# FueledByRedBull/audio-forge

Hardware: AMD Instinct MI355X
Metric: 48 kHz mono frames/s (real-time-factor x streams), voice chain (higher is better)
Workload: dtype f64

## Files before the change

audio-forge_amd/csrc/af_api.cpp:

```cpp
#include <hip/hip_runtime.h>

#include <algorithm>
#include <cmath>
#include <cstdio>
#include <cstdlib>
#include <cstring>
#include <limits>
#include <memory>
#include <string>
#include <utility>
#include <vector>

#include "af_api_internal.hpp"
#include "af_device.h"
#include "af_host.hpp"
#include "af_mixdown_host.hpp"
#include "af_output_writer_host.hpp"
#include "af_resampler_host.hpp"
#include "af_retune.h"
#include "af_stages.h"
#include "af_suppressor_host.hpp"
#include "af_switches.hpp"

namespace af {
// ... 327 lines not shown
    export_params(e);
    if (e->proto.limiter_enabled &&
        af::quad_kernel_dynamic_lds(e->host_params.n_eq_sections, e->proto.limiter.lookahead_samples, true) > af::kMaxLdsBytes)
      return fail(AF_ERR_UNSUPPORTED, "limiter lookahead of %d samples exceeds what the LDS-resident ring holds",
                  e->proto.limiter.lookahead_samples);
    if (e->proto.compressor_enabled && e->proto.compressor.auto_makeup_enabled) {
      if (e->host_params.comp.meter_slots <= 0)
        return fail(AF_ERR_UNSUPPORTED, "auto-makeup needs a control block that divides the 400 ms loudness window "
                                        "(e.g. 480 or 960 samples at 48 kHz) and a sample rate the meter supports");
      if (e->host_params.control_block < 64)
        return fail(AF_ERR_UNSUPPORTED, "auto-makeup needs control blocks of at least 64 samples");
    }
    if (!e->extra_presets.empty()) {
      for (const af_preset &ps : e->extra_presets) {
        if (ps.host_params.control_block != e->host_params.control_block)
          return fail(AF_ERR_INVALID_ARGUMENT, "every preset of an engine must use the same control block");
        if (ps.proto.sample_rate != e->proto.sample_rate) return fail(AF_ERR_INVALID_ARGUMENT, "presets must share the sample rate");
      }
      if (e->kernel != AF_KERNEL_AUTO && e->kernel != AF_KERNEL_PHASED && e->kernel != AF_KERNEL_STAGED)
        return fail(AF_ERR_UNSUPPORTED, "multi-preset engines run the token-ring kernel or the stage pipeline");
      const size_t n_groups = (size_t)(e->n_streams + 63) / 64;
      if (e->group_preset.size() != n_groups) e->group_preset.assign(n_groups, 0);
      e->d_group_preset.release();
      e->d_params_multi.release();
      AF_HIP(e->d_group_preset.reserve_exact(sizeof(int32_t) * n_groups));
      AF_HIP(hipMemcpy(e->d_group_preset, e->group_preset.data(), sizeof(int32_t) * n_groups, hipMemcpyHostToDevice));
      AF_HIP(e->d_params_multi.reserve_exact(sizeof(af::ChainParams) * (1 + e->extra_presets.size())));
      e->uploaded_multi.clear();
    }
    AF_HIP(e->d_params.reserve_exact(sizeof(af::ChainParams)));
    AF_HIP(e->d_params_pre.reserve_exact(sizeof(af::ChainParams)));
    AF_HIP(e->d_params_de.reserve_exact(sizeof(af::ChainParams)));
    if (!e->d_status) {
      AF_HIP(e->d_status.reserve_exact(sizeof(int32_t)));
      AF_HIP(e->d_status.keep_if(hipMemset(e->d_status, 0, sizeof(int32_t))));
    }
    int rc = upload_initial_state(e);
    if (rc) return rc;
    if (e->supp.enabled) {
      if (e->proto.sample_rate != 48000.0)
        return fail(AF_ERR_INVALID_ARGUMENT, "the RNNoise suppressor runs at 48 kHz only (rnnoise.rs:3,46)");
      AF_HIP(e->supp.reset_state(e->n_streams));
    }
    e->params_dirty = true;
    e->started = true;
    e->samples_processed = 0;
    e->pending = 0;
  }
  return AF_OK;
}

int check_device_status(af_engine *e) {
  if (!e->d_status) return AF_OK;
  int32_t st = 0;
  AF_HIP(hipMemcpy(&st, e->d_status, sizeof st, hipMemcpyDeviceToHost));
  if (st != 0)
    return fail(AF_ERR_BACKEND, "a chain kernel abandoned a stage token (device status %d); results are invalid.  (A one-launch call "
                                "waits for kernels on other streams: if something serialises dispatches, set AF_CHAIN_PERSISTENT=0.)", st);
  return AF_OK;
}

void advance_crossfades(af_engine *e, int64_t n) {
 for (int preset = 0; preset <= (int)e->extra_presets.size(); ++preset) {
  af::ChainParams &o = preset_params(e, preset);
  std::vector<af::SectionParams *> sections;
  for (int k = 0; k < o.n_eq_sections; ++k) sections.push_back(&o.eq[k]);
  if (o.flags & af::kFlagDeesser)
    for (auto &b : o.deesser.bands) {
// ... 1443 lines not shown
int af_engine_select_preset(af_engine *e, int32_t preset) {
  if (!e) return fail(AF_ERR_INVALID_ARGUMENT, "engine is null");
  if (preset < 0 || preset > (int32_t)e->extra_presets.size()) return fail(AF_ERR_INVALID_ARGUMENT, "preset %d does not exist", preset);
  e->current_preset = preset;
  return AF_OK;
}
int af_engine_assign_presets(af_engine *e, const int32_t *preset_of_group, int32_t n_groups) {
  if (!e || !preset_of_group) return fail(AF_ERR_INVALID_ARGUMENT, "null argument");
  if (n_groups != (e->n_streams + 63) / 64)
    return fail(AF_ERR_INVALID_ARGUMENT, "expected one preset index per group of 64 streams (%d), got %d", (e->n_streams + 63) / 64, n_groups);
  for (int32_t g = 0; g < n_groups; ++g)
    if (preset_of_group[g] < 0 || preset_of_group[g] > (int32_t)e->extra_presets.size())
      return fail(AF_ERR_INVALID_ARGUMENT, "group %d: preset %d does not exist", g, preset_of_group[g]);
  if (int rc = require_config(e)) return rc;
  e->group_preset.assign(preset_of_group, preset_of_group + n_groups);
  return AF_OK;
}

int af_engine_set_kernel(af_engine *e, int32_t kernel) {
  if (!e) return fail(AF_ERR_INVALID_ARGUMENT, "engine is null");
  if (kernel < AF_KERNEL_AUTO || kernel > AF_KERNEL_ROLES) return fail(AF_ERR_INVALID_ARGUMENT, "unknown kernel id %d", kernel);
  e->kernel = kernel;
  return AF_OK;
}
int af_engine_set_ring_variant(af_engine *e, int32_t waves, int32_t chunk) {
  if (!e) return fail(AF_ERR_INVALID_ARGUMENT, "engine is null");
  const int v = waves * 100 + chunk;
  if (v != 0 && v != 1604 && v != 1602 && v != 804 && v != 802 && v != 1204 && v != 1202)
    return fail(AF_ERR_INVALID_ARGUMENT, "no token-ring kernel is built for %d waves x %d-sample chunks", waves, chunk);
  e->ring_variant = v;
  return AF_OK;
}
int af_engine_last_kernel(const af_engine *e) { return e ? e->last_kernel_used : 0; }
int af_engine_set_timing_enabled(af_engine *e, int32_t on) {
  if (!e) return fail(AF_ERR_INVALID_ARGUMENT, "engine is null");
  e->timing = on != 0;
  return AF_OK;
}

static int check_evidence_blocks(const af_engine *e, int64_t n_run) {
  const int cb = e->host_params.control_block;
  const int64_t blocks = (n_run + cb - 1) / cb;
  if (n_run > 0 && (e->host_params.flags & af::kFlagCompressor) && e->host_params.comp.auto_makeup_enabled && e->has_evidence &&
      e->vad_blocks != blocks)
    return fail(AF_ERR_INVALID_ARGUMENT, "expected %lld VAD probabilities at the control cadence, got %lld",
                (long long)blocks, (long long)e->vad_blocks);
  if (n_run > 0 && gate_vad_fused(e) && e->vad_ev_blocks > 0 && e->vad_ev_blocks != blocks)
    return fail(AF_ERR_INVALID_ARGUMENT, "expected %lld VAD evidence blocks at the control cadence, got %lld", (long long)blocks,
                (long long)e->vad_ev_blocks);
  return AF_OK;
}

static bool io_resampled(const af_engine *e) { return e->rs_in || e->rs_out; }
static const char *const kStreamOnlyMessage =
    "this engine resamples its input or output (af_engine_set_io_sample_rates): use af_engine_stream_host";
static const char *const kWriterStreamOnlyMessage =
    "this engine runs the output writer (af_engine_set_output_writer): use af_engine_stream_host";
static const char *const kChannelsStreamOnlyMessage =
    "this engine takes multichannel input (af_engine_set_input_channels): use af_engine_stream_host";

struct CallArgs {
  const float *chain_in;
  float *out;
  int64_t n_samples, stream_stride;
  int32_t layout;
  hipStream_t stream;
// ... 1200 lines not shown
```

audio-forge_amd/csrc/af_device.h:

```cpp
#pragma once
#include <stdint.h>

namespace af {

constexpr int kNumBands = 10;
constexpr int kMaxSectionsPerBand = 4;
constexpr int kMaxEqSections = kNumBands * kMaxSectionsPerBand;
constexpr int kTpTaps = 32;
constexpr int kTpDelay = 20;
constexpr int kMaxLookahead = 1024;
constexpr int kTile = 64;
constexpr int kLanes = 64;
constexpr int kLdsLookaheadMax = 127;

struct BiquadCoef {
  double b0, b1, b2, a1, a2;
};

struct SectionParams {
  BiquadCoef active;
  BiquadCoef pending;
  int32_t xf_total;
  int32_t xf_remaining;
};
// ... 77 lines not shown
  kCompCurReleaseMs, kCompTargetReleaseMs, kCompReleaseCoeff, kCompSmoothedMakeup,
  kCompActivityScore, kCompActivityReliability, kCompCurrentLufs,
  kLimGain,
  kDeBroadbandEnv, kDeCurrentReduction, kDeConfidence,
  kDeBand0,
  kDeBandStride = 23,
  kEqBase = kDeBand0 + 3 * kDeBandStride,
  kF64Fixed = kEqBase
};
enum MeterField : int { kMeterV1 = 0, kMeterV2, kMeterV3, kMeterV4, kMeterPos, kMeterRing, kMeterFixed = kMeterRing };
inline int f64_field_count(int n_sections, int meter_slots = 0) {
  return kF64Fixed + 4 * n_sections + (meter_slots > 0 ? kMeterFixed + meter_slots : 0);
}

enum F32Field : int {
  kDcX1 = 0, kDcY1,
  kTpGain,
  kLimPrefix,
  kTpInHist,
  kTpOutHist = kTpInHist + kTpTaps,
  kLimRing = kTpOutHist + kTpTaps,
  kF32Fixed = kLimRing
};
inline int f32_field_count(int lookahead) { return kF32Fixed + 2 * (lookahead + 1); }

struct BlockStats {
  float input_sample_peak, output_sample_peak, tp_limiter_input_peak, output_true_peak;
  float limiter_peak_gr_db, tp_limiter_gr_db, compressor_gr_db, deesser_gr_db;
  double input_square_sum, output_square_sum;
  uint32_t tp_limited_events, non_finite_output;
  float makeup_gain_db, makeup_activity, makeup_reliability, pad;
};

struct LaunchArgs {
  const ChainParams *params;
  const int32_t *group_preset;
  double *st64;
  float *st32;
  const float *in;
  float *out;
  BlockStats *stats;
  int32_t *status;
  const BlockStats *pre_stats;
  const double *pre_power;
  const double *vad_prob;
  const int64_t *ready;
  int64_t n_samples;
  int64_t stream_stride;
  int64_t samples_before;
  int32_t n_streams;
  int32_t layout;
};

}
```

audio-forge_amd/csrc/af_ring_kernel.hip:

```cpp
#include <hip/hip_runtime.h>

#include <cstdlib>

#include <type_traits>

#include "af_dsp.h"
#include "af_switches.hpp"

namespace af {

constexpr int kTpRing = 128;
constexpr int kEqGroup = 5;
constexpr int kMaxEqGroups = kMaxEqSections / kEqGroup;

enum : int { kTokIn = 0, kTokCompA, kTokCompC, kTokCompE, kTokMeter, kTokLim, kTokTp, kTokFin, kTokEq0, kNumTokens = kTokEq0 + kMaxEqGroups };

enum : int {
  kR64PreZ1 = 0, kR64PreZ2,
  kR64ScPrevIn, kR64ScPrevOut, kR64LowEnv, kR64VoicedEnv, kR64PresenceEnv, kR64Plosive,
  kR64PeakEnvDb, kR64RmsEnvSq, kR64Gr, kR64FastEnv, kR64SlowEnv, kR64CurReleaseMs, kR64TargetReleaseMs,
  kR64ReleaseCoeff, kR64SmoothedMakeup, kR64MakeupLin,
  kR64LimGain, kR64LimGmin, kR64InSq, kR64OutSq,
  kR64Activity0, kR64Activity1, kR64Reliab0, kR64Reliab1, kR64MeterV1, kR64MeterV2, kR64MeterV3, kR64MeterV4,
  kR64MeterAcc, kR64ActScore, kR64ActReliab, kR64CurrentLufs,
  kR64Eq
};
enum : int {
  kR32DcX1 = 0, kR32DcY1, kR32TpGain, kR32LimPrefix, kR32InPeak, kR32OutPeak, kR32TpInPeak, kR32OutTp,
  kR32TpGmin, kR32TpLimited, kR32NonFinite, kR32Pad,
  kR32Tpi,
  kR32Tpo = kR32Tpi + kTpRing,
  kR32LimRing = kR32Tpo + kTpRing
};

__host__ __device__ inline size_t ring_lds_bytes(int n_sections, int lookahead, bool crossfade) {
  const size_t rows64 = kR64Eq + (crossfade ? 4 : 2) * (size_t)n_sections;
  const size_t rows32 = kR32LimRing + 2 * ((size_t)lookahead + 1);
  return 256 + rows64 * kLanes * sizeof(double) + rows32 * kLanes * sizeof(float);
}

#ifndef AF_PIN_MASK
#define AF_PIN_MASK (2 | 16 | 32 | 64)
#endif
#define AF_PIN(bit, v) do { if constexpr (((AF_PIN_MASK) & (bit)) != 0) asm volatile("" : "+v"(v)); } while (0)
constexpr int kAbortSlot = 32;
constexpr int kPatienceSlot = 33;
#ifdef AF_TOKEN_PROFILE
__shared__ unsigned g_prof[2][16][12];
__shared__ long long g_prof_acq[16];
__shared__ long long g_prof_ready[16];
#endif
__device__ __forceinline__ void unit_marker_begin(int tok) {
  if (__builtin_constant_p(tok)) asm volatile(";;#af-unit-begin %0" ::"i"(tok));
  else asm volatile(";;#af-unit-begin eq");
}
__device__ __forceinline__ void unit_marker_end(int tok) {
  if (__builtin_constant_p(tok)) asm volatile(";;#af-unit-end %0" ::"i"(tok));
  else asm volatile(";;#af-unit-end eq");
}
__device__ __forceinline__ void token_wait(int *turn_base, int tok, int q) {
  __builtin_amdgcn_sched_barrier(0);
#ifdef AF_TOKEN_PROFILE
  const long long prof_t0 = clock64();
#endif
  int spins = 0;
// ... 120 lines not shown
    }
    if (wave == 1 % kRingWaves) {
      const int mbase = kF64Fixed + 4 * P.n_eq_sections;
      const bool meter = kAuto && P.comp.meter_slots > 0;
      L64(kR64MeterV1) = meter ? a.st64[(int64_t)(mbase + kMeterV1) * NS + sc] : 0.0;
      L64(kR64MeterV2) = meter ? a.st64[(int64_t)(mbase + kMeterV2) * NS + sc] : 0.0;
      L64(kR64MeterV3) = meter ? a.st64[(int64_t)(mbase + kMeterV3) * NS + sc] : 0.0;
      L64(kR64MeterV4) = meter ? a.st64[(int64_t)(mbase + kMeterV4) * NS + sc] : 0.0;
      L64(kR64MeterAcc) = 0.0;
      L64(kR64ActScore) = a.st64[(int64_t)kCompActivityScore * NS + sc];
      L64(kR64ActReliab) = a.st64[(int64_t)kCompActivityReliability * NS + sc];
      L64(kR64CurrentLufs) = a.st64[(int64_t)kCompCurrentLufs * NS + sc];
      L64(kR64Activity0) = 0.0;
      L64(kR64Activity1) = 0.0;
      L64(kR64Reliab0) = 0.0;
      L64(kR64Reliab1) = 0.0;
    }
    if (wave == 0) {
      L64(kR64MakeupLin) = db2lin(a.st64[(int64_t)kCompSmoothedMakeup * NS + sc]);
      L64(kR64LimGmin) = 1.0;
      L64(kR64InSq) = 0.0;
      L64(kR64OutSq) = 0.0;
      L32(kR32DcX1) = a.st32[(int64_t)kDcX1 * NS + sc];
      L32(kR32DcY1) = a.st32[(int64_t)kDcY1 * NS + sc];
      L32(kR32TpGain) = a.st32[(int64_t)kTpGain * NS + sc];
      L32(kR32LimPrefix) = a.st32[(int64_t)kLimPrefix * NS + sc];
      L32(kR32InPeak) = 0.0f;
      L32(kR32OutPeak) = 0.0f;
      L32(kR32TpInPeak) = 0.0f;
      L32(kR32OutTp) = 0.0f;
      L32(kR32TpGmin) = 1.0f;
      L32(kR32TpLimited) = 0.0f;
      L32(kR32NonFinite) = 0.0f;
    }
    for (int r = wave; r < kTpTaps; r += kRingWaves) {
      const int row = (int)((n0 - kTpTaps + r) & (kTpRing - 1));
      L32(kR32Tpi + row) = a.st32[(int64_t)(kTpInHist + r) * NS + sc];
      L32(kR32Tpo + row) = out_detector ? a.st32[(int64_t)(kTpOutHist + r) * NS + sc] : 0.0f;
    }
    if (flags & kFlagLimiter)
      for (int r = wave; r < 2 * W; r += kRingWaves) L32(kR32LimRing + r) = a.st32[(int64_t)(kLimRing + r) * NS + sc];
  }
  __syncthreads();

  const int cb = P.control_block;
  const int cpb = (cb + kChunk - 1) / kChunk;
  const int64_t n_blocks = (a.n_samples + cb - 1) / cb;
  const int64_t last_len = a.n_samples - (n_blocks - 1) * cb;
  const int64_t Q = n_blocks > 0 ? (n_blocks - 1) * cpb + (last_len + kChunk - 1) / kChunk : 0;
  const float tp_ceiling = P.tp.ceiling_linear;
  const bool vec_ok = a.layout == 0 && (cb % kChunk) == 0 && (a.stream_stride % 4) == 0 && (kChunk % 2) == 0 &&
                      ((reinterpret_cast<uintptr_t>(a.in) | reinterpret_cast<uintptr_t>(a.out)) & 15) == 0;

  constexpr int64_t kAllReady = 0x7fffffffffffffffLL;
  int64_t ready_seen = a.ready ? 0 : kAllReady;
  for (int64_t q64 = wave; q64 < Q; q64 += kRingWaves) {
    const int q = (int)q64;
    const int64_t b = q64 / cpb;
    const int i = (int)(q64 - b * cpb);
    const int blk_len = (int)((a.n_samples - b * cb) < cb ? (a.n_samples - b * cb) : cb);
    const int64_t t0 = b * cb + (int64_t)i * kChunk;
    const int len = (blk_len - i * kChunk) < kChunk ? (blk_len - i * kChunk) : kChunk;
    if (t0 + len > ready_seen) {
      int spins = 0;
#ifdef AF_TOKEN_PROFILE
      const long long prof_r0 = clock64();
#endif
      for (;;) {
        ready_seen = __hip_atomic_load(a.ready, __ATOMIC_RELAXED, __HIP_MEMORY_SCOPE_AGENT);
        if (ready_seen >= t0 + len) break;
        __builtin_amdgcn_s_sleep(32);
        if ((++spins & 0xff) == 0 &&
            (spins > (1 << 22) || __hip_atomic_load(&turn[kAbortSlot], __ATOMIC_RELAXED, __HIP_MEMORY_SCOPE_WORKGROUP) != 0)) {
          __hip_atomic_store(&turn[kAbortSlot], 1, __ATOMIC_RELAXED, __HIP_MEMORY_SCOPE_WORKGROUP);
          ready_seen = kAllReady;
          break;
        }
      }
      __builtin_amdgcn_fence(__ATOMIC_ACQUIRE, "agent");
#ifdef AF_TOKEN_PROFILE
      if ((threadIdx.x & 63) == 0) g_prof_ready[threadIdx.x >> 6] += clock64() - prof_r0;
#endif
    }
    const bool first_in_block = i == 0;
    const bool last_in_block = i * kChunk + len == blk_len;
    BlockStats *row = a.stats ? &a.stats[b * NS + sc] : nullptr;

    const int nb = (int)((n0 + t0) & (kTpRing - 1));
// ... 476 lines not shown
                  m = fmaxf(m, fabsf(ring[kk * kLanes + lane]));
                  suf[kk * kLanes + lane] = m;
                }
              }
              j = jn;
              double tg = 1.0;
              if (__builtin_amdgcn_ballot_w64(peak > ceil_lin) != 0) {
                tg = peak > ceil_lin ? ceil_lin / peak : 1.0;
                asm volatile("" : "+v"(tg));
              }
              if (tg < g) {
                g = tg;
              } else {
                g = rc * g + (1.0 - rc) * tg;
              }
              gmin = fmin(gmin, g);
              const float o = (float)dclamp((double)delayed * g, -ceil_lin, ceil_lin);
              x[k] = finite_f32(o) ? o : 0.0f;
              L32(kR32Tpi + ((nb + k) & (kTpRing - 1))) = x[k];
            }
          L64(kR64LimGain) = g;
          L64(kR64LimGmin) = gmin;
          L32(kR32LimPrefix) = prefix;
          if (last_in_block && valid && row)
            row->limiter_peak_gr_db = gmin < 1.0 ? (float)(-lin2db(gmin, 1e-10)) : 0.0f;
        }
        token_pass(turn, kTokLim, q);
  #pragma unroll
        for (int k = 0; k < kChunk; ++k)
          if (kFull || k < len) {
            itp[k] = tp_observe_ring(&l32[kR32Tpi * kLanes], nb + k, lane);
            AF_PIN(8, itp[k]);
          }
      }

      if (!comp_only) {
      token_wait(turn, kTokTp, q);
      {
        double out_sq = first_in_block ? 0.0 : L64(kR64OutSq);
        float out_peak = first_in_block ? 0.0f : L32(kR32OutPeak);
        float nonfinite = first_in_block ? 0.0f : L32(kR32NonFinite);
        float tp_in_peak = 0.0f, tp_gmin = 1.0f, tp_limited = 0.0f;
        if (flags & kFlagLimiter) {
          float g = L32(kR32TpGain);
          tp_in_peak = first_in_block ? 0.0f : L32(kR32TpInPeak);
          tp_gmin = first_in_block ? 1.0f : L32(kR32TpGmin);
          tp_limited = first_in_block ? 0.0f : L32(kR32TpLimited);
          const float rel = P.tp.release_coeff;
  #pragma unroll
          for (int k = 0; k < kChunk; ++k)
            if (kFull || k < len) {
              const float delayed = L32(kR32Tpi + ((nb + k - kTpDelay) & (kTpRing - 1)));
              tp_in_peak = fmaxf(tp_in_peak, itp[k]);
              float tg = 1.0f;
              if (itp[k] > tp_ceiling) tg = fclamp((tp_ceiling * 0.999f) / itp[k], 0.0f, 1.0f);
              if (tg < g) {
                g = tg;
                tp_limited = 1.0f;
              } else {
                g = rel * g + (1.0f - rel) * tg;
              }
              tp_gmin = fminf(tp_gmin, g);
              float o = fclamp(delayed * g, -tp_ceiling, tp_ceiling);
              if (!finite_f32(o)) o = 0.0f;
              x[k] = o;
            }
          L32(kR32TpGain) = g;
          L32(kR32TpInPeak) = tp_in_peak;
          L32(kR32TpGmin) = tp_gmin;
          L32(kR32TpLimited) = tp_limited;
        }
  #pragma unroll
        for (int k = 0; k < kChunk; ++k)
          if (kFull || k < len) {
            const float o = x[k];
            float det = o;
            if (finite_f32(o)) {
              out_sq += (double)o * (double)o;
            } else {
              nonfinite = 1.0f;
              det = 0.0f;
            }
            out_peak = fmaxf(out_peak, fabsf(o));
            if (out_detector) L32(kR32Tpo + ((nb + k) & (kTpRing - 1))) = det;
          }
        L64(kR64OutSq) = out_sq;
        L32(kR32OutPeak) = out_peak;
        L32(kR32NonFinite) = nonfinite;
        if (last_in_block && valid && row) {
          row->output_square_sum = out_sq;
          row->output_sample_peak = out_peak;
          row->non_finite_output = nonfinite != 0.0f ? 1u : 0u;
          row->tp_limiter_input_peak = tp_in_peak;
          row->tp_limiter_gr_db =
              (flags & kFlagLimiter) && tp_gmin < 1.0f ? -20.0f * log10f(fmaxf(tp_gmin, 1e-10f)) : 0.0f;
          row->tp_limited_events = tp_limited != 0.0f ? 1u : 0u;
        }
      }
      token_pass(turn, kTokTp, q);
      }

      if (vec_ok && kFull) {
        if (valid) {
          float *dst = &a.out[(int64_t)s * a.stream_stride + t0];
          if constexpr (kChunk == 2) {
            *reinterpret_cast<float2 *>(dst) = make_float2(x[0], x[1]);
          } else {
  #pragma unroll
            for (int k4 = 0; k4 < kChunk; k4 += 4)
              *reinterpret_cast<float4 *>(dst + k4) = make_float4(x[k4], x[k4 + 1], x[k4 + 2], x[k4 + 3]);
          }
        }
      } else {
  #pragma unroll
        for (int k = 0; k < kChunk; ++k)
          if (valid && (kFull || k < len)) {
            if (a.layout == 0) a.out[(int64_t)s * a.stream_stride + t0 + k] = x[k];
            else a.out[(t0 + k) * a.stream_stride + s] = x[k];
          }
      }
      float otp = 0.0f;
      if (out_detector) {
  #pragma unroll
        for (int k = 0; k < kChunk; ++k)
          if (kFull || k < len) otp = fmaxf(otp, tp_observe_ring(&l32[kR32Tpo * kLanes], nb + k, lane));
        AF_PIN(16, otp);
      }
      if (out_detector) {
        token_wait(turn, kTokFin, q);
        {
          const float m = fmaxf(first_in_block ? 0.0f : L32(kR32OutTp), otp);
          L32(kR32OutTp) = m;
          if (last_in_block && valid && row) row->output_true_peak = m;
        }
        token_pass(turn, kTokFin, q);
      }
    };
    if (len == kChunk) chunk_body(std::true_type{});
    else chunk_body(std::false_type{});
  }
  __syncthreads();
  if (tid == 0 && turn[kAbortSlot] != 0 && a.status) atomicExch(a.status, 1);
#ifdef AF_TOKEN_PROFILE
  if (tid == 0 && blockIdx.x == 0 && Q > 0) {
    const long long ticks = clock64() - prof_k0, wall = wall_clock64() - prof_w0;
    printf("ring profile: %lld chunks, kernel %lld ticks = %.1f per chunk, %.3f ms wall, clock %.3f GHz\n", (long long)Q, ticks,
           (double)ticks / (double)Q, (double)wall * 1e-5, (double)ticks / ((double)wall * 10.0));
    if (a.ready) {
      long long r = 0;
      for (int k = 0; k < kRingWaves; ++k) r += g_prof_ready[k];
      printf("  waiting for the ready counter: %.3f ms per wave (wave 0: %.3f ms)\n",
             (double)r / kRingWaves / ((double)ticks / ((double)wall * 1e-5)), (double)g_prof_ready[0] / ((double)ticks / ((double)wall * 1e-5)));
    }
    for (int t = 0; t < kTokEq0 + n_groups; ++t) {
      long long w = 0, h = 0;
      for (int k = 0; k < kRingWaves; ++k) { w += g_prof[0][k][t]; h += g_prof[1][k][t]; }
      printf("  token %2d: held %.1f ticks per chunk, waited for %.1f\n", t, (double)h / (double)Q, (double)w / (double)Q);
    }
  }
#endif

  if (valid && (flags & kFlagPrePass)) {
    for (int k = wave; k < (any_xf ? 4 : 2) * nsec; k += kRingWaves) {
      const int sec = k >> (any_xf ? 2 : 1), part = k & (any_xf ? 3 : 1);
      const int row = part < 2 ? kR64Eq + 2 * sec + part : pz_base + 2 * sec + (part - 2);
      a.st64[(int64_t)(kEqBase + 4 * sec + part) * NS + s] = L64(row);
    }
    if (wave == 0 && (flags & kFlagDcBlock)) {
      a.st64[(int64_t)kPreZ1 * NS + s] = L64(kR64PreZ1);
      a.st64[(int64_t)kPreZ2 * NS + s] = L64(kR64PreZ2);
      a.st32[(int64_t)kDcX1 * NS + s] = L32(kR32DcX1);
      a.st32[(int64_t)kDcY1 * NS + s] = L32(kR32DcY1);
    }
  } else if (valid) {
    struct Map { int row, field; };
// ... 23 lines not shown
    }
    {
      for (int k = wave; k < n_tail64; k += kRingWaves)
        if (k > 0 || !comp_only) a.st64[(int64_t)tail64[k].field * NS + s] = L64(tail64[k].row);
      if (wave == 1 % kRingWaves && kAuto && P.comp.meter_slots > 0) {
        const int mbase = kF64Fixed + 4 * P.n_eq_sections;
        a.st64[(int64_t)(mbase + kMeterV1) * NS + s] = L64(kR64MeterV1);
        a.st64[(int64_t)(mbase + kMeterV2) * NS + s] = L64(kR64MeterV2);
        a.st64[(int64_t)(mbase + kMeterV3) * NS + s] = L64(kR64MeterV3);
        a.st64[(int64_t)(mbase + kMeterV4) * NS + s] = L64(kR64MeterV4);
      }
      if (wave == 0) {
        const double tau = fmax(L64(kR64CurReleaseMs), 0.001) / 1000.0;
        a.st64[(int64_t)kCompReleaseCoeff * NS + s] =
            P.comp.adaptive_release ? exp(-1.0 / (tau * P.comp.sample_rate)) : L64(kR64ReleaseCoeff);
        if (!(flags & kFlagCompressor)) a.st64[(int64_t)kCompGr * NS + s] = 0.0;
        if (!comp_only) {
          a.st32[(int64_t)kTpGain * NS + s] = L32(kR32TpGain);
          a.st32[(int64_t)kLimPrefix * NS + s] = L32(kR32LimPrefix);
        }
      }
      const int64_t n_end = n0 + a.n_samples;
      for (int r = wave; r < (comp_only ? 0 : kTpTaps); r += kRingWaves) {
        const int rowi = (int)((n_end - kTpTaps + r) & (kTpRing - 1));
        a.st32[(int64_t)(kTpInHist + r) * NS + s] = L32(kR32Tpi + rowi);
        if (out_detector) a.st32[(int64_t)(kTpOutHist + r) * NS + s] = L32(kR32Tpo + rowi);
      }
      if (flags & kFlagLimiter)
        for (int r = wave; r < 2 * W; r += kRingWaves) a.st32[(int64_t)(kLimRing + r) * NS + s] = L32(kR32LimRing + r);
    }
  }
#undef L64
#undef L32
}

size_t ring_kernel_dynamic_lds(int n_sections, int lookahead_samples, bool crossfade) {
  return ring_lds_bytes(n_sections, lookahead_samples, crossfade);
}

#ifdef AF_TOKEN_PROFILE
constexpr int kRingMaxDynamicLds = 160 * 1024 - 4096;
#else
constexpr int kRingMaxDynamicLds = 160 * 1024;
#endif
template <int kRingWaves, int kChunk, bool kAuto = false>
static hipError_t launch_variant(const LaunchArgs &args, size_t dyn, hipStream_t stream) {
  const int groups = (args.n_streams + kLanes - 1) / kLanes;
  static bool attr_set = false;
  if (!attr_set) {
    hipError_t err = hipFuncSetAttribute(reinterpret_cast<const void *>(chain_ring_kernel<kRingWaves, kChunk, kAuto>),
                                         hipFuncAttributeMaxDynamicSharedMemorySize, kRingMaxDynamicLds);
    if (err != hipSuccess) return err;
    attr_set = true;
  }
  hipLaunchKernelGGL((chain_ring_kernel<kRingWaves, kChunk, kAuto>), dim3(groups), dim3(kRingWaves * kLanes), dyn, stream,
                     args, args.params);
  return hipGetLastError();
}

hipError_t launch_chain_ring_lds(const LaunchArgs &args, size_t dyn, int variant, bool auto_makeup, hipStream_t stream);
hipError_t launch_chain_ring(const LaunchArgs &args, int n_sections, int lookahead_samples, bool crossfade, int variant,
                             bool auto_makeup, hipStream_t stream) {
  return launch_chain_ring_lds(args, ring_lds_bytes(n_sections, lookahead_samples, crossfade), variant, auto_makeup, stream);
}
__global__ void chain_publish_ready_kernel(int64_t *ready, int64_t samples) {
  __hip_atomic_store(ready, samples, __ATOMIC_RELEASE, __HIP_MEMORY_SCOPE_AGENT);
// ... 27 lines not shown
```

audio-forge_amd/mic_eq_mi/_lib.py:

```python
from __future__ import annotations

import ctypes as C
import pathlib

PKG_DIR = pathlib.Path(__file__).resolve().parents[1]
import os

LIB_PATH = pathlib.Path(os.environ.get("AF_LIB_PATH") or (PKG_DIR / "libaudioforge_mi.so"))

AF_OK = 0
AF_ERR_INVALID_ARGUMENT = -1
AF_ERR_BACKEND = -2
AF_ERR_NON_FINITE = -3
AF_ERR_STATE = -4
AF_ERR_UNSUPPORTED = -5

LAYOUT_STREAM_MAJOR = 0
LAYOUT_TIME_MAJOR = 1
KERNEL_AUTO, KERNEL_LANE_PER_STREAM, KERNEL_PHASED, KERNEL_QUAD, KERNEL_STAGED, KERNEL_ROLES = 0, 1, 2, 3, 4, 5


class EqBandConfig(C.Structure):
    _fields_ = [
        ("filter_type", C.c_int32),
# ... 366 lines not shown
    "af_noise_suppressor_backend_failed": (_i32, [_vp]),
    "af_noise_suppressor_backend_error": (C.c_char_p, [_vp]),
    "af_engine_last_block_count": (_i64, [_vp]),
    "af_engine_read_block_stats": (C.c_int, [_vp, C.POINTER(BlockStats), _i64]),
    "af_engine_samples_processed": (_i64, [_vp]),
    "af_engine_set_preset_count": (C.c_int, [_vp, _i32]),
    "af_engine_preset_count": (_i32, [_vp]),
    "af_engine_select_preset": (C.c_int, [_vp, _i32]),
    "af_engine_assign_presets": (C.c_int, [_vp, C.POINTER(_i32), _i32]),
    "af_engine_set_kernel": (C.c_int, [_vp, _i32]),
    "af_engine_set_ring_variant": (C.c_int, [_vp, _i32, _i32]),
    "af_engine_set_timing_enabled": (C.c_int, [_vp, _i32]),
    "af_engine_last_kernel_ms": (C.c_int, [_vp, _dp, C.POINTER(_i32)]),
    "af_engine_last_stage_ms": (C.c_int, [_vp, _dp, _dp]),
    "af_engine_set_gate_enabled": (C.c_int, [_vp, _i32]),
    "af_gate_set_threshold": (C.c_int, [_vp, _d]),
    "af_gate_set_attack_time": (C.c_int, [_vp, _d]),
    "af_gate_set_release_time": (C.c_int, [_vp, _d]),
    "af_gate_set_mode": (C.c_int, [_vp, _i32]),
    "af_gate_threshold_db": (_d, [_vp]),
    "af_engine_gate_enabled": (_i32, [_vp]),
    "af_engine_read_gate_state": (C.c_int, [_vp, _fp, C.POINTER(C.c_uint64), C.POINTER(_i32), _i32]),
    "af_gate_set_vad_auto_gate_enabled": (C.c_int, [_vp, _i32]),
    "af_gate_set_vad_threshold": (C.c_int, [_vp, _d]),
    "af_gate_set_hold_time": (C.c_int, [_vp, _d]),
    "af_gate_set_margin": (C.c_int, [_vp, _d]),
    "af_gate_set_auto_threshold": (C.c_int, [_vp, _i32]),
    "af_gate_read_vad_controls": (C.c_int, [_vp, _dp, _dp, _dp, C.POINTER(_i32), C.POINTER(_i32)]),
    "af_gate_set_vad_evidence": (C.c_int, [_vp, _fp, C.POINTER(C.c_uint8), _i64, _i32]),
    "af_engine_read_gate_vad_decisions": (C.c_int, [_vp, _fp, _fp, C.POINTER(_i32), _i64]),
    "af_engine_read_gate_vad_state": (C.c_int, [_vp, _fp, _fp, _fp, _fp, C.POINTER(_i32), C.POINTER(_i32), _i32]),
    "af_engine_last_chain_launch_ms": (C.c_int, [_vp, _dp, _dp, C.POINTER(_i32)]),
    "af_engine_last_kernel": (C.c_int, [_vp]),
    "af_resampler_calculate_cutoff": (C.c_int, [_i32, _i32, C.POINTER(C.c_float)]),
    "af_resampler_create": (C.c_int, [C.c_uint32, C.c_uint32, _i64, _i32, _i32, _i32, C.POINTER(_vp)]),
    "af_resampler_destroy": (None, [_vp]),
    "af_resampler_output_delay": (C.c_int, [_vp]),
    "af_resampler_expected_frames": (_i64, [_vp, _i64]),
    "af_resampler_sinc_len": (C.c_int, [_vp]),
    "af_resampler_copy_sinc_table": (C.c_int, [_vp, _dp]),
    "af_resampler_plan": (C.c_int, [_vp, _i64, C.POINTER(_i64), C.POINTER(_i64)]),
    "af_resampler_process_device": (C.c_int, [_vp, _vp, _vp, _i64, _i32, _i64, _i64, _vp]),
    "af_resampler_process_host": (C.c_int, [_vp, _dp, _dp, _i64, _i32, _i64, _i64]),
    "af_resampler_last_kernel_ms": (C.c_int, [_vp, _dp]),
    "af_resampler_launch_form": (C.c_int, [_vp, C.POINTER(_i32), C.POINTER(_i32), C.POINTER(_i32)]),
    "af_stream_resampler_create": (C.c_int, [C.c_uint32, C.c_uint32, _i64, _i32, _i32, _i32, _i32, C.POINTER(_vp)]),
    "af_stream_resampler_destroy": (None, [_vp]),
    "af_stream_resampler_push_host": (C.c_int, [_vp, _fp, _i64, _i64, _fp, _i64, _i64, C.POINTER(_i64)]),
    "af_stream_resampler_push_device": (C.c_int, [_vp, _vp, _i64, _i64, _vp, _i64, _i64, C.POINTER(_i64), _vp]),
    "af_stream_resampler_output_frames": (_i64, [_vp, _i64]),
    "af_stream_resampler_pending_input": (_i64, [_vp]),
    "af_stream_resampler_output_delay": (C.c_int, [_vp]),
    "af_stream_resampler_frames_in": (_i64, [_vp]),
    "af_stream_resampler_frames_out": (_i64, [_vp]),
    "af_stream_resampler_reset": (C.c_int, [_vp]),
    "af_stream_resampler_clear_pending": (C.c_int, [_vp]),
    "af_stream_resampler_last_kernel_ms": (C.c_int, [_vp, _dp]),
    "af_stream_resampler_launch_form": (C.c_int, [_vp, C.POINTER(_i32), C.POINTER(_i32), C.POINTER(_i32)]),
    "af_engine_set_io_sample_rates": (C.c_int, [_vp, C.c_uint32, C.c_uint32]),
    "af_engine_stream_plan": (C.c_int, [_vp, _i64, C.POINTER(_i64), C.POINTER(_i64), C.POINTER(_i64)]),
    "af_engine_io_resampler_delay": (C.c_int, [_vp, C.POINTER(_i32), C.POINTER(_i32)]),
    "af_engine_io_resampler_pending": (C.c_int, [_vp, C.POINTER(_i64), C.POINTER(_i64)]),
    "af_mixdown_create": (C.c_int, [_i32, _i32, _i32, _i32, C.POINTER(_vp)]),
    "af_mixdown_destroy": (None, [_vp]),
    "af_mixdown_set_mode": (C.c_int, [_vp, _i32]),
    "af_mixdown_mode": (_i32, [_vp]),
# ... 200 lines not shown
```

audio-forge_amd/mic_eq_mi/mic_eq_core.py:

```python
from __future__ import annotations

import ctypes as C
import dataclasses
import time
from typing import Any, Mapping, Sequence

import numpy as np

from . import _lib
from ._lib import BlockStats, EqBandConfig

NUM_BANDS = 10
EQ_TYPE_IDS = {"low_shelf": 0, "bell": 1, "high_shelf": 2, "notch": 3, "high_pass": 4, "low_pass": 5}
CAREFUL_OUTPUT_CEILING_DB = -1.5
STATS_DTYPE = np.dtype(
    [
        ("input_sample_peak", "<f4"),
        ("output_sample_peak", "<f4"),
        ("true_peak_limiter_input_peak", "<f4"),
        ("output_true_peak", "<f4"),
        ("limiter_peak_gain_reduction_db", "<f4"),
        ("true_peak_limiter_gain_reduction_db", "<f4"),
        ("compressor_gain_reduction_db", "<f4"),
        ("deesser_gain_reduction_db", "<f4"),
# ... 254 lines not shown
    def gate_vad_controls(self) -> dict:
        thr, hold, margin = C.c_double(0.0), C.c_double(0.0), C.c_double(0.0)
        auto, attached = C.c_int32(0), C.c_int32(0)
        _lib.check(self._lib.af_gate_read_vad_controls(self._h, C.byref(thr), C.byref(hold), C.byref(margin), C.byref(auto),
                                                        C.byref(attached)))
        return {"vad_threshold": thr.value, "hold_ms": hold.value, "margin_db": margin.value,
                "auto_threshold": bool(auto.value), "attached": bool(attached.value)}

    def gate_vad_decisions(self, n_blocks: int) -> dict:
        prob = np.zeros((n_blocks, self.n_streams), dtype=np.float32)
        floor = np.zeros((n_blocks, self.n_streams), dtype=np.float32)
        flags = np.zeros((n_blocks, self.n_streams), dtype=np.int32)
        fp = C.POINTER(C.c_float)
        _lib.check(self._lib.af_engine_read_gate_vad_decisions(self._h, prob.ctypes.data_as(fp), floor.ctypes.data_as(fp),
                                                                flags.ctypes.data_as(C.POINTER(C.c_int32)), int(n_blocks)))
        return {"probability": prob, "noise_floor_db": floor, "held_open": (flags & 1) != 0, "available": (flags & 4) != 0}

    def gate_vad_state(self) -> dict:
        f = [np.zeros(self.n_streams, dtype=np.float32) for _ in range(4)]
        state = np.zeros(self.n_streams, dtype=np.int32)
        flags = np.zeros(self.n_streams, dtype=np.int32)
        fp, ip = C.POINTER(C.c_float), C.POINTER(C.c_int32)
        _lib.check(self._lib.af_engine_read_gate_vad_state(self._h, *(x.ctypes.data_as(fp) for x in f), state.ctypes.data_as(ip),
                                                            flags.ctypes.data_as(ip), self.n_streams))
        return {"noise_floor_db": f[0], "noise_floor_reliability": f[1], "fused_score": f[2], "probability": f[3],
                "gate_state": state, "held_open": (flags & 1) != 0, "fused_open": (flags & 2) != 0, "available": (flags & 4) != 0}

    def block_stats(self) -> np.ndarray:
        blocks = int(self._lib.af_engine_last_block_count(self._h))
        rows = np.zeros((blocks, self.n_streams), dtype=STATS_DTYPE)
        if blocks:
            _lib.check(self._lib.af_engine_read_block_stats(self._h, rows.ctypes.data_as(C.POINTER(BlockStats)), rows.size))
        return rows

    def last_kernel_ms(self) -> tuple[float, int]:
        ms, launches = C.c_double(0.0), C.c_int32(0)
        _lib.check(self._lib.af_engine_last_kernel_ms(self._h, C.byref(ms), C.byref(launches)))
        return ms.value, launches.value

    def last_chain_launch_ms(self) -> tuple[float, float, int]:
        first, tail, segments = C.c_double(0.0), C.c_double(0.0), C.c_int32(0)
        _lib.check(self._lib.af_engine_last_chain_launch_ms(self._h, C.byref(first), C.byref(tail), C.byref(segments)))
        return first.value, tail.value, segments.value


def _audio_1d(audio) -> np.ndarray:
    if not isinstance(audio, np.ndarray) or audio.dtype != np.float32 or audio.ndim != 1:
        raise TypeError("audio must be a 1-D numpy.float32 array")
    if not audio.flags.c_contiguous:
        raise ValueError("audio must be a contiguous float32 array")
    return audio


def _bands_v2(bands, sample_rate: float):
    if not np.isfinite(sample_rate) or sample_rate <= 0.0:
        raise ValueError("sample_rate must be finite and positive")
    if len(bands) != NUM_BANDS:
        raise ValueError(f"expected {NUM_BANDS} EQ bands, got {len(bands)}")
    arr = (EqBandConfig * NUM_BANDS)()
    lib = _lib.load()
    for index, (name, freq, gain, q, slope, enabled) in enumerate(bands):
        if name not in EQ_TYPE_IDS:
            raise ValueError(f"band {index} has unsupported EQ filter type: {name}")
        arr[index] = EqBandConfig(EQ_TYPE_IDS[name], float(freq), float(gain), float(q), int(slope), int(bool(enabled)))
        _lib.check(lib.af_eq_band_config_validate(C.byref(arr[index]), index, float(sample_rate)))
    return arr
# ... 2100 lines not shown
```

include/audioforge_mi.h:

```cpp
#ifndef AUDIOFORGE_MI_H
#define AUDIOFORGE_MI_H

#include <stddef.h>
#include <stdint.h>

#ifdef __cplusplus
extern "C" {
#endif

typedef enum af_status {
  AF_OK = 0,
  AF_ERR_INVALID_ARGUMENT = -1,
  AF_ERR_BACKEND = -2,
  AF_ERR_NON_FINITE = -3,
  AF_ERR_STATE = -4,
  AF_ERR_UNSUPPORTED = -5
} af_status;

typedef struct af_engine af_engine;

enum { AF_EQ_LOW_SHELF = 0, AF_EQ_BELL = 1, AF_EQ_HIGH_SHELF = 2, AF_EQ_NOTCH = 3,
       AF_EQ_HIGH_PASS = 4, AF_EQ_LOW_PASS = 5 };

typedef struct af_eq_band_config {
// ... 118 lines not shown
int af_limiter_set_lookahead_ms(af_engine *e, double lookahead_ms);
double af_limiter_ceiling_db(const af_engine *e);
int32_t af_limiter_lookahead_samples(const af_engine *e);

int af_true_peak_limiter_set_release_ms(af_engine *e, float release_ms);

int af_deesser_set_auto_enabled(af_engine *e, int32_t enabled);
int af_deesser_set_auto_amount(af_engine *e, double amount);
int af_deesser_set_low_cut_hz(af_engine *e, double hz);
int af_deesser_set_high_cut_hz(af_engine *e, double hz);
int af_deesser_set_threshold_db(af_engine *e, double db);
int af_deesser_set_ratio(af_engine *e, double ratio);
int af_deesser_set_attack_ms(af_engine *e, double ms);
int af_deesser_set_release_ms(af_engine *e, double ms);
int af_deesser_set_max_reduction_db(af_engine *e, double db);

int af_engine_process_device(af_engine *e, const float *in, float *out, int64_t n_samples,
                             int64_t stream_stride, int32_t layout, void *hip_stream);
int af_engine_process_host(af_engine *e, const float *in, float *out, int64_t n_samples,
                           int32_t layout);
int af_engine_synchronize(af_engine *e);
int af_engine_stream_host(af_engine *e, const float *in, int64_t n_in, float *out, int64_t out_stride, int64_t *n_out);
int64_t af_engine_pending_input(const af_engine *e);
int64_t af_engine_last_output_samples(const af_engine *e);
int64_t af_engine_last_block_count(const af_engine *e);
int af_engine_read_block_stats(af_engine *e, af_block_stats *out, int64_t capacity);
int64_t af_engine_samples_processed(const af_engine *e);
int af_engine_set_preset_count(af_engine *e, int32_t n);
int32_t af_engine_preset_count(const af_engine *e);
int af_engine_select_preset(af_engine *e, int32_t preset);
int af_engine_assign_presets(af_engine *e, const int32_t *preset_of_group, int32_t n_groups);
int af_engine_set_kernel(af_engine *e, int32_t kernel);
int af_engine_last_kernel(const af_engine *e);
int af_engine_set_ring_variant(af_engine *e, int32_t waves, int32_t chunk);
int af_engine_set_timing_enabled(af_engine *e, int32_t enabled);
int af_engine_last_kernel_ms(af_engine *e, double *ms, int32_t *launches);
int af_engine_last_stage_ms(af_engine *e, double *suppressor_ms, double *chain_ms);
int af_engine_last_chain_launch_ms(af_engine *e, double *first_ms, double *tail_ms, int32_t *segments);

typedef struct af_resampler af_resampler;
enum { AF_WINDOW_BLACKMAN_HARRIS = 0, AF_WINDOW_BLACKMAN_HARRIS_SQUARED = 1, AF_WINDOW_BLACKMAN = 2,
       AF_WINDOW_BLACKMAN_SQUARED = 3, AF_WINDOW_HANN = 4, AF_WINDOW_HANN_SQUARED = 5 };
int af_resampler_calculate_cutoff(int32_t sinc_len, int32_t window, float *out);
int af_resampler_create(uint32_t input_rate, uint32_t output_rate, int64_t chunk_size, int32_t sinc_len,
                        int32_t window, int32_t device, af_resampler **out);
void af_resampler_destroy(af_resampler *r);
int af_resampler_output_delay(const af_resampler *r);
int64_t af_resampler_expected_frames(const af_resampler *r, int64_t n_in);
int af_resampler_sinc_len(const af_resampler *r);
int af_resampler_copy_sinc_table(const af_resampler *r, double *out);
int af_resampler_plan(af_resampler *r, int64_t n_in, int64_t *n_out, int64_t *blocks);
int af_resampler_process_device(af_resampler *r, const double *d_in, double *d_out, int64_t n_in,
                                int32_t n_streams, int64_t in_stride, int64_t out_stride, void *hip_stream);
int af_resampler_process_host(af_resampler *r, const double *in, double *out, int64_t n_in, int32_t n_streams,
                              int64_t in_stride, int64_t out_stride);
int af_resampler_last_kernel_ms(af_resampler *r, double *ms);
int af_resampler_launch_form(const af_resampler *r, int32_t *form, int32_t *segment_outputs,
                             int32_t *streams_per_workgroup);

typedef struct af_stream_resampler af_stream_resampler;
int af_stream_resampler_create(uint32_t input_rate, uint32_t output_rate, int64_t chunk_size, int32_t sinc_len,
                               int32_t window, int32_t n_streams, int32_t device, af_stream_resampler **out);
void af_stream_resampler_destroy(af_stream_resampler *r);
int af_stream_resampler_push_host(af_stream_resampler *r, const float *in, int64_t n_in, int64_t in_stride, float *out,
                                  int64_t out_capacity, int64_t out_stride, int64_t *n_out);
int af_stream_resampler_push_device(af_stream_resampler *r, const float *d_in, int64_t n_in, int64_t in_stride,
// ... 612 lines not shown
```

Before: 12.82 billion.

## Reuse input true-peak detector maxima for output detector when true-peak limiter is transparent

When the true-peak stage leaves samples bit-identical for a long enough run (tracked per lane as a clean-chunk counter), the output true-peak detector result equals the input detector's maximum delayed by the true-peak delay. The kernel stores per-chunk input oversampled maxima in a small LDS ring and, when the whole wave is clean, reads the delayed max instead of recomputing the 32-tap oversampled output detector. A reuse counter is added to the status buffer with a debug API. This adds LDS traffic, a ballot, an LDS atomic per reused chunk and extra bookkeeping in the serial token section.

```diff
diff --git a/audio-forge_amd/csrc/af_api.cpp b/audio-forge_amd/csrc/af_api.cpp
--- a/audio-forge_amd/csrc/af_api.cpp
+++ b/audio-forge_amd/csrc/af_api.cpp
@@ -383,8 +383,8 @@
     AF_HIP(e->d_params_pre.reserve_exact(sizeof(af::ChainParams)));
     AF_HIP(e->d_params_de.reserve_exact(sizeof(af::ChainParams)));
     if (!e->d_status) {
-      AF_HIP(e->d_status.reserve_exact(sizeof(int32_t)));
-      AF_HIP(e->d_status.keep_if(hipMemset(e->d_status, 0, sizeof(int32_t))));
+      AF_HIP(e->d_status.reserve_exact(sizeof(int32_t) * af::kStatusWords));
+      AF_HIP(e->d_status.keep_if(hipMemset(e->d_status, 0, sizeof(int32_t) * af::kStatusWords)));
     }
     int rc = upload_initial_state(e);
     if (rc) return rc;
@@ -1894,6 +1894,17 @@
   return AF_OK;
 }
 int af_engine_last_kernel(const af_engine *e) { return e ? e->last_kernel_used : 0; }
+int af_engine_debug_detector_reuse_chunks(af_engine *e, uint64_t *chunks) {
+  if (!e || !chunks) return fail(AF_ERR_INVALID_ARGUMENT, "null argument");
+  *chunks = 0;
+  if (!e->d_status) return AF_OK;
+  AF_HIP(e->use_device());
+  AF_HIP(hipDeviceSynchronize());
+  unsigned long long n = 0;
+  AF_HIP(hipMemcpy(&n, e->d_status.get() + af::kStatusReuseWord, sizeof n, hipMemcpyDeviceToHost));
+  *chunks = (uint64_t)n;
+  return AF_OK;
+}
 int af_engine_set_timing_enabled(af_engine *e, int32_t on) {
   if (!e) return fail(AF_ERR_INVALID_ARGUMENT, "engine is null");
   e->timing = on != 0;
diff --git a/audio-forge_amd/csrc/af_device.h b/audio-forge_amd/csrc/af_device.h
--- a/audio-forge_amd/csrc/af_device.h
+++ b/audio-forge_amd/csrc/af_device.h
@@ -133,6 +133,7 @@
   float makeup_gain_db, makeup_activity, makeup_reliability, pad;
 };
 
+constexpr int kStatusWords = 4, kStatusReuseWord = 2;
 struct LaunchArgs {
   const ChainParams *params;
   const int32_t *group_preset;
diff --git a/audio-forge_amd/csrc/af_ring_kernel.hip b/audio-forge_amd/csrc/af_ring_kernel.hip
--- a/audio-forge_amd/csrc/af_ring_kernel.hip
+++ b/audio-forge_amd/csrc/af_ring_kernel.hip
@@ -12,6 +12,12 @@
 constexpr int kTpRing = 128;
 constexpr int kEqGroup = 5;
 constexpr int kMaxEqGroups = kMaxEqSections / kEqGroup;
+constexpr int kDetDelayChunks = kTpDelay / 4;
+constexpr int kDetCleanChunks = (kTpTaps - 1 + 3) / 4 + 1;
+constexpr float kDetCleanCap = 15.0f;
+constexpr int kItpMaxRing = 24;
+static_assert(kTpDelay % 4 == 0 && kDetCleanChunks == 9 && kDetCleanCap >= kDetCleanChunks,
+              "detector reuse: delay in whole chunks, clean run within its cap");
 
 enum : int { kTokIn = 0, kTokCompA, kTokCompC, kTokCompE, kTokMeter, kTokLim, kTokTp, kTokFin, kTokEq0, kNumTokens = kTokEq0 + kMaxEqGroups };
 
@@ -27,10 +33,13 @@
 };
 enum : int {
   kR32DcX1 = 0, kR32DcY1, kR32TpGain, kR32LimPrefix, kR32InPeak, kR32OutPeak, kR32TpInPeak, kR32OutTp,
-  kR32TpGmin, kR32TpLimited, kR32NonFinite, kR32Pad,
+  kR32TpGmin, kR32TpLimited, kR32NonFinite,
+  kR32TpClean,
+  kR32ReuseCount,
   kR32Tpi,
   kR32Tpo = kR32Tpi + kTpRing,
-  kR32LimRing = kR32Tpo + kTpRing
+  kR32ItpMax = kR32Tpo + kTpRing,
+  kR32LimRing = kR32ItpMax + kItpMaxRing
 };
 
 __host__ __device__ inline size_t ring_lds_bytes(int n_sections, int lookahead, bool crossfade) {
@@ -217,6 +226,8 @@
       L32(kR32TpGmin) = 1.0f;
       L32(kR32TpLimited) = 0.0f;
       L32(kR32NonFinite) = 0.0f;
+      L32(kR32TpClean) = 0.0f;
+      L32(kR32ReuseCount) = 0.0f;
     }
     for (int r = wave; r < kTpTaps; r += kRingWaves) {
       const int row = (int)((n0 - kTpTaps + r) & (kTpRing - 1));
@@ -239,6 +250,13 @@
 
   constexpr int64_t kAllReady = 0x7fffffffffffffffLL;
   int64_t ready_seen = a.ready ? 0 : kAllReady;
+#ifdef AF_NO_DETECTOR_REUSE
+  constexpr bool kDetReuse = false;
+#else
+  constexpr bool kDetReuse = kChunk == 4;
+  static_assert(!kDetReuse || kItpMaxRing >= kRingWaves + kDetDelayChunks, "a row of chunk maxima is read before its next writer starts");
+#endif
+#define AF_DET_REUSE (kDetReuse && out_detector && (flags & kFlagLimiter) != 0)
   for (int64_t q64 = wave; q64 < Q; q64 += kRingWaves) {
     const int q = (int)q64;
     const int64_t b = q64 / cpb;
@@ -781,8 +799,15 @@
             itp[k] = tp_observe_ring(&l32[kR32Tpi * kLanes], nb + k, lane);
             AF_PIN(8, itp[k]);
           }
-      }
-
+        if (kFull && AF_DET_REUSE) {
+          float m = 0.0f;
+  #pragma unroll
+          for (int k = 0; k < kChunk; ++k) m = fmaxf(m, itp[k]);
+          L32(kR32ItpMax + q % kItpMaxRing) = m;
+        }
+      }
+
+      float clean_run = 0.0f;
       if (!comp_only) {
       token_wait(turn, kTokTp, q);
       {
@@ -791,6 +816,7 @@
         float nonfinite = first_in_block ? 0.0f : L32(kR32NonFinite);
         float tp_in_peak = 0.0f, tp_gmin = 1.0f, tp_limited = 0.0f;
         if (flags & kFlagLimiter) {
+          unsigned changed = kFull ? 0u : 1u;
           float g = L32(kR32TpGain);
           tp_in_peak = first_in_block ? 0.0f : L32(kR32TpInPeak);
           tp_gmin = first_in_block ? 1.0f : L32(kR32TpGmin);
@@ -813,7 +839,12 @@
               float o = fclamp(delayed * g, -tp_ceiling, tp_ceiling);
               if (!finite_f32(o)) o = 0.0f;
               x[k] = o;
+              if (kDetReuse) changed |= __float_as_uint(o) ^ __float_as_uint(delayed);
             }
+          if (kDetReuse) {
+            clean_run = changed == 0u ? fminf(L32(kR32TpClean) + 1.0f, kDetCleanCap) : 0.0f;
+            L32(kR32TpClean) = clean_run;
+          }
           L32(kR32TpGain) = g;
           L32(kR32TpInPeak) = tp_in_peak;
           L32(kR32TpGmin) = tp_gmin;
@@ -869,7 +900,11 @@
           }
       }
       float otp = 0.0f;
-      if (out_detector) {
+      if (kFull && AF_DET_REUSE && __builtin_amdgcn_ballot_w64(clean_run < (float)kDetCleanChunks) == 0) {
+        otp = L32(kR32ItpMax + (q - kDetDelayChunks) % kItpMaxRing);
+        atomicAdd(reinterpret_cast<unsigned *>(&L32(kR32ReuseCount)), 1u);
+        AF_PIN(16, otp);
+      } else if (out_detector) {
   #pragma unroll
         for (int k = 0; k < kChunk; ++k)
           if (kFull || k < len) otp = fmaxf(otp, tp_observe_ring(&l32[kR32Tpo * kLanes], nb + k, lane));
@@ -889,7 +924,11 @@
     else chunk_body(std::false_type{});
   }
   __syncthreads();
-  if (tid == 0 && turn[kAbortSlot] != 0 && a.status) atomicExch(a.status, 1);
+  if (tid == 0 && a.status) {
+    if (turn[kAbortSlot] != 0) atomicExch(a.status, 1);
+    const unsigned reused = *reinterpret_cast<const unsigned *>(&L32(kR32ReuseCount));
+    if (kDetReuse && reused != 0) atomicAdd(reinterpret_cast<unsigned long long *>(a.status + kStatusReuseWord), (unsigned long long)reused);
+  }
 #ifdef AF_TOKEN_PROFILE
   if (tid == 0 && blockIdx.x == 0 && Q > 0) {
     const long long ticks = clock64() - prof_k0, wall = wall_clock64() - prof_w0;
@@ -979,6 +1018,7 @@
   }
 #undef L64
 #undef L32
+#undef AF_DET_REUSE
 }
 
 size_t ring_kernel_dynamic_lds(int n_sections, int lookahead_samples, bool crossfade) {
diff --git a/audio-forge_amd/mic_eq_mi/_lib.py b/audio-forge_amd/mic_eq_mi/_lib.py
--- a/audio-forge_amd/mic_eq_mi/_lib.py
+++ b/audio-forge_amd/mic_eq_mi/_lib.py
@@ -422,6 +422,7 @@
     "af_engine_read_gate_vad_state": (C.c_int, [_vp, _fp, _fp, _fp, _fp, C.POINTER(_i32), C.POINTER(_i32), _i32]),
     "af_engine_last_chain_launch_ms": (C.c_int, [_vp, _dp, _dp, C.POINTER(_i32)]),
     "af_engine_last_kernel": (C.c_int, [_vp]),
+    "af_engine_debug_detector_reuse_chunks": (C.c_int, [_vp, C.POINTER(C.c_uint64)]),
     "af_resampler_calculate_cutoff": (C.c_int, [_i32, _i32, C.POINTER(C.c_float)]),
     "af_resampler_create": (C.c_int, [C.c_uint32, C.c_uint32, _i64, _i32, _i32, _i32, C.POINTER(_vp)]),
     "af_resampler_destroy": (None, [_vp]),
diff --git a/audio-forge_amd/mic_eq_mi/mic_eq_core.py b/audio-forge_amd/mic_eq_mi/mic_eq_core.py
--- a/audio-forge_amd/mic_eq_mi/mic_eq_core.py
+++ b/audio-forge_amd/mic_eq_mi/mic_eq_core.py
@@ -310,6 +310,11 @@
         if blocks:
             _lib.check(self._lib.af_engine_read_block_stats(self._h, rows.ctypes.data_as(C.POINTER(BlockStats)), rows.size))
         return rows
+
+    def debug_detector_reuse_chunks(self) -> int:
+        n = C.c_uint64(0)
+        _lib.check(self._lib.af_engine_debug_detector_reuse_chunks(self._h, C.byref(n)))
+        return int(n.value)
 
     def last_kernel_ms(self) -> tuple[float, int]:
         ms, launches = C.c_double(0.0), C.c_int32(0)
diff --git a/include/audioforge_mi.h b/include/audioforge_mi.h
--- a/include/audioforge_mi.h
+++ b/include/audioforge_mi.h
@@ -174,6 +174,7 @@
 int af_engine_assign_presets(af_engine *e, const int32_t *preset_of_group, int32_t n_groups);
 int af_engine_set_kernel(af_engine *e, int32_t kernel);
 int af_engine_last_kernel(const af_engine *e);
+int af_engine_debug_detector_reuse_chunks(af_engine *e, uint64_t *chunks);
 int af_engine_set_ring_variant(af_engine *e, int32_t waves, int32_t chunk);
 int af_engine_set_timing_enabled(af_engine *e, int32_t enabled);
 int af_engine_last_kernel_ms(af_engine *e, double *ms, int32_t *launches);
```

Measured after the change: 12.99 billion (median of 6 runs). +1.3%, better.
